# ishine/ASR-Rescoring

Hardware: AMD Instinct MI355X
Metric: masked-token BERT forwards/sec (MLM_PLL, N=50, L~32) (higher is better)
Workload: dtype fp16x3-split (fp32-accurate: hi/lo fp16 operand split on fp16 MFMA, fp32 accumulate)

## Files before the change

asr-rescoring_amd/csrc/gemm_dev.h:

```cpp
#pragma once
#include "common.h"

namespace {

typedef float f32x2 __attribute__((ext_vector_type(2)));
__device__ __forceinline__ f32x2 gelu2(f32x2 x) {
    constexpr float AMAX = 8.06101731f;
    const f32x2 a = __builtin_elementwise_min(__builtin_elementwise_abs(x), (f32x2)(AMAX));
    f32x2 q = __builtin_elementwise_fma(a, (f32x2)(3.309473686e-05f), (f32x2)(-7.692362997e-04f));
    q = __builtin_elementwise_fma(q, a, (f32x2)(8.080770262e-03f));
    q = __builtin_elementwise_fma(q, a, (f32x2)(-5.341218412e-02f));
    q = __builtin_elementwise_fma(q, a, (f32x2)(-4.587709010e-01f));
    q = __builtin_elementwise_fma(q, a, (f32x2)(-1.151201725e+00f));
    q = __builtin_elementwise_fma(q, a, (f32x2)(-9.999930859e-01f));
    const f32x2 e = {__builtin_amdgcn_exp2f(q.x), __builtin_amdgcn_exp2f(q.y)};
    const f32x2 r = x - __builtin_elementwise_min(x, (f32x2)(0.f));
    return __builtin_elementwise_fma(-a, e, r);
}

template <int E>
__device__ __forceinline__ float mix_val(unsigned hi2, unsigned lo2, float inv64) {
    float d;
    if constexpr (E == 0)
        asm("v_fma_mix_f32 %0, %1, %2, %3 op_sel_hi:[1,0,1]" : "=v"(d) : "v"(lo2), "s"(inv64), "v"(hi2));
    else
        asm("v_fma_mix_f32 %0, %1, %2, %3 op_sel:[1,0,1] op_sel_hi:[1,0,1]" : "=v"(d) : "v"(lo2), "s"(inv64), "v"(hi2));
    return d;
}
__device__ __forceinline__ unsigned mix_lo2(unsigned hi2, float x0x64, float x1x64, float neg64) {
    unsigned d;
    asm("v_fma_mixlo_f16 %0, %1, %2, %3 op_sel_hi:[1,0,0]" : "=v"(d) : "v"(hi2), "s"(neg64), "v"(x0x64));
    asm("v_fma_mixhi_f16 %0, %1, %2, %3 op_sel:[1,0,0] op_sel_hi:[1,0,0]" : "+v"(d) : "v"(hi2), "s"(neg64), "v"(x1x64));
    return d;
}

template <bool NT>
__device__ __forceinline__ void st16(uint4* p, uint4 v) {
    typedef unsigned int u32x4 __attribute__((ext_vector_type(4)));
    if constexpr (NT) __builtin_nontemporal_store((u32x4){v.x, v.y, v.z, v.w}, (u32x4*)p);
    else *p = v;
}

__device__ __forceinline__ int g16(int rb) { return (0x78 >> (2 * (rb & 3))) & 3; }

__device__ __forceinline__ void slab_read4(const char* slb, int rr0, int c16, uint4 (&v)[4]) {
    const uint32_t base = (uint32_t)(uintptr_t)(const __attribute__((address_space(3))) char*)slb;
    uint32_t a[4];
#pragma unroll
    for (int it = 0; it < 4; ++it) {
        const int rr = it * 8 + rr0;
        a[it] = base + rr * 128 + ((c16 ^ (rr & 7)) << 4);
    }
    uint4 v0, v1, v2, v3;
    asm volatile(
        "ds_read_b128 %0, %4\n\t"
        "ds_read_b128 %1, %5\n\t"
        "ds_read_b128 %2, %6\n\t"
        "ds_read_b128 %3, %7\n\t"
        "s_waitcnt lgkmcnt(0)"
        : "=&v"(v0), "=&v"(v1), "=&v"(v2), "=&v"(v3)
        : "v"(a[0]), "v"(a[1]), "v"(a[2]), "v"(a[3])
        : "memory");
    v[0] = v0; v[1] = v1; v[2] = v2; v[3] = v3;
}

}
```

asr-rescoring_amd/csrc/k_gemm.hip:

```cpp
#include <atomic>
#include "common.h"
#include "gemm_dev.h"

#ifndef RS_DIAG
#define RS_DIAG 0
#endif
#include <stdio.h>
#include <stdlib.h>
#include <string.h>
#include <type_traits>

namespace {

enum : int {
    P_SCHED = 1 << 18,
    P_SLAB = 1 << 20,
    P_X3IMG = 1 << 22,
    P_TAG_OPROJ = 1 << 16,
    P_TAG_FFN2 = 1 << 17,
    X_GANG_XCD = 1 << 27,
    X_TAG_FFN2 = 1 << 26,
    X_DIAG_NOSTAGE = 1,
    X_DIAG_NOSTORE = 2,
    X_DIAG_NOWAIT = 8,
// ... 674 lines not shown

__device__ __forceinline__ unsigned long long lnr_wait_ticks(int diag) { return (diag & 8) ? 1000ull : 100000000ull; }
__device__ __forceinline__ unsigned long long lnr_form_ticks(int diag) { return (diag & 8) ? 1000ull : 1000000000ull; }
__device__ __forceinline__ unsigned long long lnr_now() { return __builtin_amdgcn_s_memrealtime(); }

typedef __attribute__((address_space(1))) unsigned lgu32;
typedef __attribute__((address_space(1))) unsigned long long lgu64;
__device__ __forceinline__ unsigned lnr_add(unsigned* c, int w, unsigned v = 1u) {
    return __hip_atomic_fetch_add((lgu32*)(c + w), v, __ATOMIC_RELAXED, __HIP_MEMORY_SCOPE_AGENT);
}
__device__ __forceinline__ unsigned lnr_ld(const unsigned* c, int w) {
    return __hip_atomic_load((const lgu32*)(c + w), __ATOMIC_RELAXED, __HIP_MEMORY_SCOPE_AGENT);
}

constexpr unsigned LNR_PENDING = 0xfffffffeu, LNR_CANCELLED = 0xffffffffu;
constexpr unsigned long long LNR_CANCEL_TICKS = 5000ull;
template <bool XCD>
__device__ unsigned lnr_gang_ticket(const EpiArgs& ep, int ntn_, int n_panels) {
    unsigned* c = ep.lncnt;
    const unsigned ntn = (unsigned)ntn_, G = gridDim.x;
    const unsigned long long tag = (unsigned long long)ep.ln_tag << 32;
    unsigned long long* tab = (unsigned long long*)c + LNC_TAB;
    const unsigned long long t_lim = lnr_form_ticks(ep.diag), t_start = lnr_now();
    auto ld64 = [](unsigned long long* p) {
        return __hip_atomic_load((const lgu64*)p, __ATOMIC_RELAXED, __HIP_MEMORY_SCOPE_AGENT);
    };
    auto cas64 = [](unsigned long long* p, unsigned long long& expect, unsigned long long want) {
        return __hip_atomic_compare_exchange_strong((lgu64*)p, &expect, want, __ATOMIC_RELAXED, __ATOMIC_RELAXED,
                                                    __HIP_MEMORY_SCOPE_AGENT);
    };
    const unsigned NL = min(G / ntn, (unsigned)n_panels);
    auto exhausted = [&]() { return lnr_ld(c, LNC_GANGS) >= NL; };
    auto complete = [&](unsigned long long* slot, unsigned& gid) -> bool {
        unsigned long long v = ld64(slot);
        for (;;) {
            if ((v >> 32) == (tag >> 32)) return false;
            if (cas64(slot, v, tag | LNR_PENDING)) break;
        }
        gid = lnr_add(c, LNC_GANGS);
        __hip_atomic_store((lgu64*)slot, tag | gid, __ATOMIC_RELAXED, __HIP_MEMORY_SCOPE_AGENT);
        return true;
    };
    auto await_id = [&](unsigned long long* slot, bool local, unsigned& gid) -> int {
        const unsigned long long t0 = lnr_now();
        for (unsigned spins = 1;; ++spins) {
            unsigned long long v = ld64(slot);
            if ((v >> 32) == (tag >> 32)) {
                const unsigned st = (unsigned)v;
                if (st == LNR_CANCELLED) return -1;
                if (st != LNR_PENDING) {
                    gid = st;
                    return 1;
                }
            } else if ((local && lnr_now() - t0 > ((ep.diag & 8) ? 0ull : LNR_CANCEL_TICKS)) || exhausted()) {
                if (cas64(slot, v, tag | LNR_CANCELLED)) return -1;
                continue;
            }
            if ((spins & 63) == 0 && (lnr_now() - t_start > t_lim || lnr_ld(ep.lnerr, 0))) return 0;
            __builtin_amdgcn_s_sleep(1);
        }
    };
    unsigned gid = 0, mem = 0;
    bool ovf = !XCD, ok = true;
    if constexpr (XCD) {
        unsigned x;
        asm volatile("s_getreg_b32 %0, hwreg(HW_REG_XCC_ID)" : "=s"(x));
        x &= 7;
        const unsigned cap = (G / 8) / ntn * ntn;
        const unsigned lc = lnr_add(c, LNC_LOCAL + 16 * (int)x);
        ovf = lc >= cap;
        if (!ovf) {
            const unsigned k = lc / ntn;
            mem = lc - k * ntn;
            unsigned long long* slot = tab + x * 128 + k;
            if (mem + 1 == ntn) {
                ovf = !complete(slot, gid);
            } else {
                const int r = await_id(slot, true, gid);
                ok = r != 0;
                ovf = r < 0;
            }
        }
    }
    if (ovf && ok) {
        const unsigned o = lnr_add(c, LNC_OVF), k = o / ntn;
        mem = o - k * ntn;
        unsigned long long* slot = tab + 8 * 128 + k;
        if (k >= 256) {
            ok = false;
        } else if (mem + 1 == ntn) {
            if (!complete(slot, gid)) gid = NL;
        } else {
            const int r = await_id(slot, false, gid);
            ok = r != 0;
            if (r < 0) gid = NL;
        }
    }
    if (!ok) {
        __hip_atomic_store((lgu32*)ep.lnerr, 1u, __ATOMIC_RELAXED, __HIP_MEMORY_SCOPE_AGENT);
        return 0xffffffffu;
    }
    return gid >= NL ? 0xfffffffeu : gid * ntn + mem;
}

__device__ __forceinline__ bool lnr_next_list(const EpiArgs& ep, int& t, unsigned nlist, int p, int tcol, int ntn,
                                              int n_tiles, int wave, int lane) {
    const int n_panels = n_tiles / ntn;
    const unsigned NL = min((unsigned)(gridDim.x / ntn), (unsigned)n_panels);
    const unsigned long long tag = (unsigned long long)ep.ln_tag << 32;
    unsigned long long* clm = (unsigned long long*)ep.lnx + (size_t)n_panels * ntn * 512 + p;
    if (tcol == 0 && wave == 0 && lane == 0)
        __hip_atomic_store((lgu64*)clm, tag | nlist, __ATOMIC_RELAXED, __HIP_MEMORY_SCOPE_AGENT);
    const unsigned long long t_lim = lnr_wait_ticks(ep.diag), t_start = lnr_now();
    for (unsigned spins = 1;; ++spins) {
        const unsigned long long v = __hip_atomic_load((const lgu64*)clm, __ATOMIC_RELAXED, __HIP_MEMORY_SCOPE_AGENT);
        if ((v >> 32) == (tag >> 32) && !(ep.diag & 8)) {
            const unsigned l = (unsigned)v;
            t = l < NL ? (int)l * ntn + tcol : n_tiles;
            return true;
        }
        if ((spins & 63) == 0 && (lnr_now() - t_start > t_lim || lnr_ld(ep.lnerr, 0))) {
            if (lane == 0) __hip_atomic_store((lgu32*)ep.lnerr, 1u, __ATOMIC_RELAXED, __HIP_MEMORY_SCOPE_AGENT);
            return false;
        }
        __builtin_amdgcn_s_sleep(1);
    }
}

__device__ __forceinline__ void lnr_done(const EpiArgs& ep, int lane) {
    unsigned* c = ep.lncnt;
    unsigned last = 0;
    if (lane == 0) last = lnr_add(c, LNC_DONE) + 1 == gridDim.x;
    if (!__builtin_amdgcn_readfirstlane(last)) return;
    static_assert(LNC_TAB_N % 64 == 0, "gang slots per lane");
    unsigned long long* tab = (unsigned long long*)c + LNC_TAB;
#pragma unroll
    for (int i = 0; i < LNC_TAB_N / 64; ++i)
        __hip_atomic_store((lgu64*)(tab + lane + 64 * i), 0ull, __ATOMIC_RELAXED, __HIP_MEMORY_SCOPE_AGENT);
    if (lane != 0) return;
    const int w[] = {LNC_OVF, LNC_GANGS, LNC_DONE};
    for (int x = 0; x < 8; ++x) __hip_atomic_store((lgu32*)(c + LNC_LOCAL + 16 * x), 0u, __ATOMIC_RELAXED, __HIP_MEMORY_SCOPE_AGENT);
    for (int i = 0; i < 3; ++i) __hip_atomic_store((lgu32*)(c + w[i]), 0u, __ATOMIC_RELAXED, __HIP_MEMORY_SCOPE_AGENT);
}

template <int EPI, int OPT>
__global__ void __launch_bounds__(512)
gemm_x3s_kernel(const f16* __restrict__ A, const f16* __restrict__ W, int K, int ldw, int n_tiles_n, int n_tiles,
                EpiArgs ep) {
    constexpr int BM = 256, BK = 32, NW = 8, WN = 4, WTM = 128, WTN = 64;
    constexpr int RB = BK * 2;
    constexpr int REG = BM * RB;
    constexpr int STAGE = 4 * REG;
    constexpr int NSTORE = 32;
    static_assert(EPI == EPI_BIAS_F32 || EPI == EPI_GELU_F16 || EPI == EPI_LNRES_IMG, "x3s epilogues");
    constexpr bool LNR = EPI == EPI_LNRES_IMG;
    constexpr int DV = RS_DIAG ? OPT & (X_DIAG_NOSTAGE | X_DIAG_NOSTORE | X_DIAG_NOWAIT | X_DIAG_PANEL0 | X_DIAG_STAMP) : 0;
    static_assert(!LNR || (DV & X_DIAG_NOSTORE) == 0, "the LayerNorm epilogue has no no-store diagnostic");
    constexpr bool STAMP = (DV & X_DIAG_STAMP) != 0;
    unsigned long long st_sum[10] = {0, 0, 0, 0, 0, 0, 0, 0, 0, 0}, st_prev = 0;
    auto stamp = [&](int ph) __attribute__((always_inline)) {
        if constexpr (STAMP) {
            unsigned long long tt;
            __builtin_amdgcn_sched_barrier(0);
            asm volatile("s_memtime %0\n\ts_waitcnt lgkmcnt(0)" : "=s"(tt)::"memory");
            __builtin_amdgcn_sched_barrier(0);
            if (ph >= 0) st_sum[ph] += tt - st_prev;
            st_prev = tt;
        }
    };
    stamp(-1);
    extern __shared__ __attribute__((aligned(16))) char smem[];
    __shared__ __attribute__((aligned(16))) char slabs[NW * 4096];

    const int tid = threadIdx.x, lane = tid & 63;
    const int wave = __builtin_amdgcn_readfirstlane(tid >> 6);
    const int wm = wave / WN, wn = wave % WN;
    const int nk = K / BK;
    int t = blockIdx.x;
    typedef __attribute__((address_space(1))) unsigned gu32;
    typedef __attribute__((address_space(1))) unsigned long long gu64;
    if constexpr (LNR) {
        if (tid == 0) *(unsigned*)(slabs + 2048) = lnr_gang_ticket<(OPT & X_GANG_XCD) != 0>(ep, n_tiles_n, n_tiles / n_tiles_n);
        __syncthreads();
        t = (int)*(const unsigned*)(slabs + 2048);
    }
    stamp(8);
    if ((unsigned)t >= (unsigned)n_tiles) {
        if constexpr (LNR) {
            if (wave == 0) lnr_done(ep, lane);
        }
        return;
    }
    if (wave >= NW / 2) __builtin_amdgcn_s_setprio(1);
    auto tile_of = [&](int tt, int& m0, int& n0) {
        if constexpr (LNR) {
            m0 = (tt / n_tiles_n) * BM;
            n0 = (tt - (tt / n_tiles_n) * n_tiles_n) * BM;
            return;
        }
        const int xcd = tt & 7, pos = tt >> 3, q = n_tiles >> 3, r = n_tiles & 7;
        const int wgid = (xcd < r ? xcd * (q + 1) : r * (q + 1) + (xcd - r) * q) + pos;
        const int GM = ep.group_m, n_tiles_m = n_tiles / n_tiles_n, per_group = GM * n_tiles_n;
        const int g = wgid / per_group, loc = wgid - g * per_group;
        const int gm = min(GM, n_tiles_m - g * GM);
        const int tn = loc / gm;
        m0 = (g * GM + (loc - tn * gm)) * BM;
        n0 = tn * BM;
    };
    const size_t ld2 = (size_t)2 * K;
    __amdgpu_buffer_rsrc_t rsA, rsW;
    int voffA[4], voffW[4];
    auto wperm = [](int L) {
        return LNR ? (L & ~31) | (((L >> 2) & 3) << 3) | (((L >> 4) & 1) << 2) | (L & 3) : L;
    };
#pragma unroll
    for (int h = 0; h < 2; ++h)
#pragma unroll
        for (int l = 0; l < 2; ++l) {
            const int n = 128 * h + wave * 16 + 8 * l + (lane >> 3);
            const int sl = ((lane & 7) ^ ((n >> 1) & 7)) * 8;
            voffA[2 * h + l] = (n * (int)ld2 + sl) * 2;
            voffW[2 * h + l] = (wperm(n) * ldw + sl) * 2;
        }
    auto set_rsrc = [&](int m0, int n0) {
        rsA = __builtin_amdgcn_make_buffer_rsrc((void*)(A + (size_t)m0 * ld2), (short)0, (int)(256 * ld2 * 2), 0x00020000);
        rsW = __builtin_amdgcn_make_buffer_rsrc((void*)(W + (size_t)n0 * ldw), (short)0, 256 * ldw * 2, 0x00020000);
    };
    auto piece = [&](int buf, int k0, int p) {
        if constexpr ((DV & X_DIAG_NOSTAGE) != 0) return;
        const int r = p >> 1;
        const int dofs = (r >> 1) * 2 * REG + ((p & 1) * 128 + wave * 16 + 8 * (r & 1)) * 128;
        auto* dst = (__attribute__((address_space(3))) void*)(smem + buf * STAGE + dofs);
        const int vo = (r < 2 ? voffA : voffW)[2 * (p & 1) + (r & 1)];
        __builtin_amdgcn_raw_ptr_buffer_load_lds(r < 2 ? rsA : rsW, dst, 16, vo, k0 * 4, 0, 0);
    };
    auto stage = [&](int buf, int k0) {
#pragma unroll
        for (int p = 0; p < 8; ++p) piece(buf, k0, p);
    };
    const half8 up = (half8)(f16)X3_UP;

    const int r16 = lane & 15, q4 = lane >> 4;
    const int offA16 = (wm * WTM + r16) * 128 + ((q4 ^ ((r16 >> 1) & 7)) << 4);
    const int offW16 = 2 * REG + (wn * WTN + r16) * 128 + ((q4 ^ ((r16 >> 1) & 7)) << 4);
    f32x4 acc16[8][4];
    auto kstep16 = [&](int buf, int k0n) {
        const char* sb = smem + buf * STAGE;
        half8 wh[4], wl[4], wu[4];
#pragma unroll
        for (int j = 0; j < 4; ++j) {
            wh[j] = *(const half8*)(sb + offW16 + j * 2048);
            wl[j] = *(const half8*)(sb + (offW16 ^ 64) + j * 2048);
        }
#pragma unroll
        for (int j = 0; j < 4; ++j) wu[j] = wh[j] * up;
#pragma unroll
        for (int h = 0; h < 2; ++h) {
            half8 ah[4], al[4];
#pragma unroll
            for (int ii = 0; ii < 4; ++ii) {
                ah[ii] = *(const half8*)(sb + offA16 + (4 * h + ii) * 2048);
                al[ii] = *(const half8*)(sb + (offA16 ^ 64) + (4 * h + ii) * 2048);
            }
#pragma unroll
            for (int pr = 0; pr < 3; ++pr) {
#pragma unroll
                for (int ii = 0; ii < 4; ++ii) {
#pragma unroll
                    for (int j = 0; j < 4; ++j) {
                        const half8 b = pr == 0 ? wu[j] : pr == 1 ? wh[j] : wl[j];
                        const half8 a = pr == 1 ? al[ii] : ah[ii];
                        acc16[4 * h + ii][j] = __builtin_amdgcn_mfma_f32_16x16x32_f16(b, a, acc16[4 * h + ii][j], 0, 0, 0);
                    }
                    const int grp = 12 * h + 4 * pr + ii;
                    if (grp < 8 && k0n < (1 << 29)) {
                        __builtin_amdgcn_sched_barrier(0);
                        piece(buf ^ 1, k0n, grp);
                        __builtin_amdgcn_sched_barrier(0);
                    }
                }
            }
        }
    };

    int m0, n0;
    tile_of(t, m0, n0);
    set_rsrc(m0, n0);
    stage(0, 0);
    int par = 0;
    bool first = true;
    for (;;) {
        unsigned nlist = 0;
        if constexpr (LNR) {
            if (m0 / BM + (int)gridDim.x / n_tiles_n >= n_tiles / n_tiles_n && n0 == 0 && wave == 0 && lane == 0)
                nlist = lnr_add(ep.lncnt, LNC_GANGS);
        }
#pragma unroll
        for (int i = 0; i < 8; ++i)
#pragma unroll
            for (int j = 0; j < 4; ++j) acc16[i][j] = (f32x4)(0.f);
        int kt0 = 0;
        if constexpr (LNR) {
            if constexpr ((DV & X_DIAG_NOWAIT) == 0) {
                if (!first) asm volatile("s_waitcnt vmcnt(%0)" ::"n"(NSTORE) : "memory");
                else asm volatile("s_waitcnt vmcnt(0)" ::: "memory");
            }
            asm volatile("s_barrier" ::: "memory");
            __builtin_amdgcn_sched_barrier(0);
            kstep16(par, BK);
            __builtin_amdgcn_sched_barrier(0);
            stamp(9);
            kt0 = 1;
        }
        for (int kt = kt0; kt < nk; ++kt) {
            const int cur = (par + kt) & 1;
            if constexpr ((DV & X_DIAG_NOWAIT) != 0) {
            } else if (kt == 0 && !first) asm volatile("s_waitcnt vmcnt(%0)" ::"n"(NSTORE) : "memory");
            else asm volatile("s_waitcnt vmcnt(0)" ::: "memory");
            asm volatile("s_barrier" ::: "memory");
            __builtin_amdgcn_sched_barrier(0);
            kstep16(cur, kt + 1 < nk ? (kt + 1) * BK : (1 << 29));
            __builtin_amdgcn_sched_barrier(0);
            if constexpr (STAMP && !LNR) {
                if (kt == 0) stamp(9);
            }
        }
        stamp(0);
        const int last = (par + nk - 1) & 1;
        const int cm0 = m0, cn0 = n0;
        const int rbo = (last ^ 1) * STAGE + wave * 8192;
        const __amdgpu_buffer_rsrc_t rsR = __builtin_amdgcn_make_buffer_rsrc(
            (void*)((const f16*)ep.out + (size_t)cm0 * ep.ldc), (short)0, 256 * ep.ldc * 2, 0x00020000);
        int voR[4];
#pragma unroll
        for (int q = 0; q < 4; ++q) {
            const int jr = 8 * (q & 1) + (lane >> 3);
            const int cc = (lane & 7) ^ ((jr >> 1) & 7);
            voR[q] = ((wm * WTM + jr) * ep.ldc + 2 * (cn0 + wn * WTN) + 64 * (q >> 1) + 8 * cc) * 2;
        }
        auto issue = [&](int rb) __attribute__((always_inline)) {
#pragma unroll
            for (int q = 0; q < 4; ++q) {
                auto* dst = (__attribute__((address_space(3))) void*)(smem + rbo + (rb & 1) * 4096 + q * 1024);
                __builtin_amdgcn_raw_ptr_buffer_load_lds(rsR, dst, 16, voR[q], rb * 16 * ep.ldc * 2, 0, 0);
            }
        };
        if constexpr (LNR) {
            issue(0);
            issue(1);
        }
        f32x4 bq[4];
#pragma unroll
        for (int j = 0; j < 4; ++j) {
            const float* bp = ep.bias + cn0 + wn * WTN + (LNR ? 32 * (j >> 1) + 8 * q4 + 4 * (j & 1) : 16 * j + 4 * q4);
            asm volatile("global_load_dwordx4 %0, %1, off" : "=v"(bq[j]) : "v"(bp) : "memory");
        }
        asm volatile("s_waitcnt vmcnt(0)" : "+v"(bq[0]), "+v"(bq[1]), "+v"(bq[2]), "+v"(bq[3]) : : "memory");
        bool more = false;
        t += gridDim.x;
        if constexpr (LNR) {
            if (t >= n_tiles && !lnr_next_list(ep, t, nlist, cm0 / BM, cn0 / BM, n_tiles_n, n_tiles, wave, lane)) break;
        }
        more = t < n_tiles;
        if (more) {
            tile_of(t, m0, n0);
            set_rsrc(m0, n0);
            if constexpr (!LNR) stage(last ^ 1, 0);
        }
        stamp(1);
        auto finish = [&](int i0, int i1) {
#pragma unroll
            for (int i = i0; i < i1; ++i)
#pragma unroll
                for (int j = 0; j < 4; ++j)
#pragma unroll
                    for (int e = 0; e < 4; e += 2) {
                        f32x2 v = __builtin_elementwise_fma((f32x2){acc16[i][j][e], acc16[i][j][e + 1]}, (f32x2)(X3_DOWN),
                                                            (f32x2){bq[j][e], bq[j][e + 1]});
                        if constexpr (EPI == EPI_GELU_F16) v = gelu2(v);
                        acc16[i][j][e] = v.x;
                        acc16[i][j][e + 1] = v.y;
                    }
        };
            auto lnres_epilogue = [&]() {
                const int H = ep.nlog, ntn = n_tiles_n;
                const int panel = cm0 / BM, tcol = cn0 / BM;
                const unsigned long long tag = (unsigned long long)ep.ln_tag << 32;
                auto add_res = [&](int rb, const half4 (&rh)[4], const half4 (&rl)[4]) __attribute__((always_inline)) {
#pragma unroll
                    for (int j = 0; j < 4; ++j) {
                        const uint2 hv = __builtin_bit_cast(uint2, rh[j]), lv = __builtin_bit_cast(uint2, rl[j]);
                        const float hres[4] = {mix_val<0>(hv.x, lv.x, X3_DOWN), mix_val<1>(hv.x, lv.x, X3_DOWN),
                                               mix_val<0>(hv.y, lv.y, X3_DOWN), mix_val<1>(hv.y, lv.y, X3_DOWN)};
#pragma unroll
                        for (int e = 0; e < 4; ++e)
                            acc16[rb][j][e] = __builtin_fmaf(acc16[rb][j][e], X3_DOWN, bq[j][e]) + hres[e];
                    }
                };
                {
                    const uint32_t lrow = (uint32_t)(uintptr_t)(const __attribute__((address_space(3))) char*)smem + rbo +
                                          r16 * 128;
                    const uint32_t lh = lrow + ((q4 ^ ((r16 >> 1) & 7)) << 4), ll = lrow + (((q4 + 4) ^ ((r16 >> 1) & 7)) << 4);
#pragma unroll
                    for (int rb = 0; rb < 8; ++rb) {
                        if (rb < 7) asm volatile("s_waitcnt vmcnt(4)" ::: "memory");
                        else asm volatile("s_waitcnt vmcnt(0)" ::: "memory");
                        uint4 h0, h1, l0, l1;
                        const int so = (rb & 1) * 4096;
                        asm volatile(
                            "ds_read_b128 %0, %4 offset:%6\n\t"
                            "ds_read_b128 %1, %4 offset:%7\n\t"
                            "ds_read_b128 %2, %5 offset:%6\n\t"
                            "ds_read_b128 %3, %5 offset:%7\n\t"
                            "s_waitcnt lgkmcnt(0)"
                            : "=&v"(h0), "=&v"(h1), "=&v"(l0), "=&v"(l1)
                            : "v"(lh), "v"(ll), "i"(so), "i"(so + 2048)
                            : "memory");
                        if (rb + 2 < 8) issue(rb + 2);
                        const half8 vh0 = __builtin_bit_cast(half8, h0), vh1 = __builtin_bit_cast(half8, h1);
                        const half8 vl0 = __builtin_bit_cast(half8, l0), vl1 = __builtin_bit_cast(half8, l1);
                        const half4 rh[4] = {(half4){vh0[0], vh0[1], vh0[2], vh0[3]}, (half4){vh0[4], vh0[5], vh0[6], vh0[7]},
                                             (half4){vh1[0], vh1[1], vh1[2], vh1[3]}, (half4){vh1[4], vh1[5], vh1[6], vh1[7]}};
                        const half4 rl[4] = {(half4){vl0[0], vl0[1], vl0[2], vl0[3]}, (half4){vl0[4], vl0[5], vl0[6], vl0[7]},
                                             (half4){vl1[0], vl1[1], vl1[2], vl1[3]}, (half4){vl1[4], vl1[5], vl1[6], vl1[7]}};
                        add_res(rb, rh, rl);
                    }
                }
                stamp(2);
                float* red = (float*)(slabs + wave * 4096);
                auto slab_of = [&](int w2) { return (const float*)(slabs + (wm * WN + w2) * 4096); };
                float tmean[8];
#pragma unroll
                for (int i = 0; i < 8; ++i) {
                    float a = 0.f;
#pragma unroll
                    for (int j = 0; j < 4; ++j) a += (acc16[i][j][0] + acc16[i][j][1]) + (acc16[i][j][2] + acc16[i][j][3]);
                    a += __shfl_xor(a, 16);
                    a += __shfl_xor(a, 32);
                    tmean[i] = a;
                }
                if (q4 == 0) {
#pragma unroll
                    for (int i = 0; i < 8; ++i) red[16 * i + r16] = tmean[i];
                }
                asm volatile("s_waitcnt lgkmcnt(0)\n\ts_barrier" ::: "memory");
#pragma unroll
                for (int i = 0; i < 8; ++i) {
                    float a = 0.f;
#pragma unroll
                    for (int w2 = 0; w2 < WN; ++w2) a += slab_of(w2)[16 * i + r16];
                    tmean[i] = a * (1.f / BM);
                }
#pragma unroll
                for (int i = 0; i < 8; ++i) {
                    float q = 0.f;
#pragma unroll
                    for (int j = 0; j < 4; ++j)
#pragma unroll
                        for (int e = 0; e < 4; ++e) {
                            const float d = acc16[i][j][e] - tmean[i];
                            q = __builtin_fmaf(d, d, q);
                        }
                    q += __shfl_xor(q, 16);
                    q += __shfl_xor(q, 32);
                    if (q4 == 0) red[128 + 16 * i + r16] = q;
                }
                asm volatile("s_waitcnt lgkmcnt(0)\n\ts_barrier" ::: "memory");
                float2* st2 = (float2*)(smem + last * STAGE) + wm * WTM;
                volatile unsigned* bailw = (volatile unsigned*)(smem + last * STAGE + 4096);
                if (wn == 0) {
                    typedef unsigned long long u64;
                    u64* gx = (u64*)ep.lnx + (size_t)panel * ntn * BM * 2 + wm * WTM * 2;
                    int ln = lane;
                    asm volatile("" : "+v"(ln));
                    float os[2], oq[2];
#pragma unroll
                    for (int k = 0; k < 2; ++k) {
                        const int rr = ln + 64 * k;
                        float a = 0.f, b = 0.f;
#pragma unroll
                        for (int w2 = 0; w2 < WN; ++w2) {
                            a += slab_of(w2)[rr];
                            b += slab_of(w2)[128 + rr];
                        }
                        os[k] = a;
                        oq[k] = b;
                        u64* g = gx + ((size_t)tcol * BM + rr) * 2;
                        __hip_atomic_store((gu64*)g, tag | __float_as_uint(a), __ATOMIC_RELAXED, __HIP_MEMORY_SCOPE_AGENT);
                        __hip_atomic_store((gu64*)(g + 1), tag | __float_as_uint(b), __ATOMIC_RELAXED, __HIP_MEMORY_SCOPE_AGENT);
                    }
                    float ps[2][4], pq[2][4];
                    bool failed = false;
                    stamp(3);
                    const unsigned long long t_lim = lnr_wait_ticks(ep.diag), t_start = lnr_now();
                    for (unsigned spins = 0;;) {
                        bool ok = true;
#pragma unroll
                        for (int k = 0; k < 2; ++k)
#pragma unroll
                            for (int c = 0; c < 4; ++c) {
                                ps[k][c] = os[k];
                                pq[k][c] = oq[k];
                                if (c < ntn && c != tcol) {
                                    const u64* g = gx + ((size_t)c * BM + ln + 64 * k) * 2;
                                    const u64 va = __hip_atomic_load((const gu64*)g, __ATOMIC_RELAXED, __HIP_MEMORY_SCOPE_AGENT);
                                    const u64 vb = __hip_atomic_load((const gu64*)(g + 1), __ATOMIC_RELAXED, __HIP_MEMORY_SCOPE_AGENT);
                                    ok &= (va >> 32) == (tag >> 32) && (vb >> 32) == (tag >> 32);
                                    ps[k][c] = __uint_as_float((unsigned)va);
                                    pq[k][c] = __uint_as_float((unsigned)vb);
                                }
                            }
                        if (ep.diag & 8) ok = false;
                        if (__all(ok)) break;
                        __builtin_amdgcn_s_sleep(1);
                        if ((++spins & 63) == 0 &&
                            (lnr_now() - t_start > t_lim ||
                             __hip_atomic_load((const gu32*)ep.lnerr, __ATOMIC_RELAXED, __HIP_MEMORY_SCOPE_AGENT))) {
                            if (lane == 0) __hip_atomic_store((gu32*)ep.lnerr, 1u, __ATOMIC_RELAXED, __HIP_MEMORY_SCOPE_AGENT);
                            failed = true;
                            break;
                        }
                    }
#pragma unroll
                    for (int k = 0; k < 2; ++k) {
                        const float inv_n = 1.f / H;
                        float tot = 0.f;
#pragma unroll
                        for (int c = 0; c < 4; ++c)
                            if (c < ntn) tot += ps[k][c];
                        const float mean = tot * inv_n;
                        float m2 = 0.f;
#pragma unroll
                        for (int c = 0; c < 4; ++c) {
                            if (c < ntn) {
                                const float d = ps[k][c] * (1.f / BM) - mean;
                                m2 += __builtin_fmaf((float)BM * d, d, pq[k][c]);
                            }
                        }
                        st2[lane + 64 * k] = make_float2(mean, 1.0f / sqrtf(__builtin_fmaf(m2, inv_n, ep.ln_eps)));
                    }
                    if (lane == 0) bailw[wm] = failed ? 1u : 0u;
                    stamp(4);
                }
                asm volatile("s_waitcnt lgkmcnt(0)\n\ts_barrier" ::: "memory");
                if (bailw[0] | bailw[1]) return true;
                f32x4 gq[4], bb[4];
#pragma unroll
                for (int j = 0; j < 4; ++j) {
                    const int cj = cn0 + wn * WTN + 32 * (j >> 1) + 8 * q4 + 4 * (j & 1);
                    gq[j] = *(const f32x4*)(ep.res_g + cj);
                    bb[j] = *(const f32x4*)(ep.res_b + cj);
                }
#pragma unroll
                for (int i = 0; i < 8; ++i) {
                    const float2 st = st2[16 * i + r16];
#pragma unroll
                    for (int j = 0; j < 4; ++j)
#pragma unroll
                        for (int e = 0; e < 4; ++e) acc16[i][j][e] = ln_apply(acc16[i][j][e], st, gq[j][e], bb[j][e]);
                }
                stamp(5);
                return false;
            };
            constexpr bool LATE = EPI == EPI_GELU_F16 && (DV & X_DIAG_NOSTORE) == 0;
            if constexpr (LNR) {
                if (lnres_epilogue()) {
                    asm volatile("s_waitcnt vmcnt(0)" ::: "memory");
                    break;
                }
                if (more) stage(last ^ 1, 0);
            } else if constexpr (!LATE) finish(0, 8);
            if constexpr ((DV & X_DIAG_NOSTORE) != 0) {
#pragma unroll
                for (int i = 0; i < 8; ++i)
#pragma unroll
                    for (int j = 0; j < 4; ++j) asm volatile("" ::"v"(acc16[i][j]));
                if (!more) break;
                par = last ^ 1;
                first = false;
                continue;
            }
            char* slb = slabs + wave * 4096;
            int lns = lane;
            if constexpr (LNR) asm volatile("" : "+v"(lns));
            const int rr0 = lns >> 3, c16 = lns & 7;
            const int sm0 = (DV & X_DIAG_PANEL0) ? 0 : cm0;
            if constexpr (EPI == EPI_BIAS_F32) {
#pragma unroll
                for (int i2 = 0; i2 < 4; ++i2)
#pragma unroll
                    for (int j2 = 0; j2 < 2; ++j2) {
#pragma unroll
                        for (int a = 0; a < 2; ++a)
#pragma unroll
                            for (int b = 0; b < 2; ++b) {
                                const int row = 16 * a + r16, ch = 4 * b + q4;
                                *(f32x4*)(slb + row * 128 + ((ch ^ (row & 7)) << 4)) = acc16[2 * i2 + a][2 * j2 + b];
                            }
                        float* ob = (float*)ep.out + (size_t)(sm0 + wm * WTM + 32 * i2) * ep.ldc + cn0 + wn * WTN + 32 * j2 + 4 * c16;
                        uint4 v[4];
                        slab_read4(slb, rr0, c16, v);
#pragma unroll
                        for (int it = 0; it < 4; ++it) st16<true>((uint4*)(ob + (size_t)(it * 8 + rr0) * ep.ldc), v[it]);
                    }
            } else {
#pragma unroll
                for (int i2 = 0; i2 < 4; ++i2) {
                    if constexpr (LATE) finish(2 * i2, 2 * i2 + 2);
#pragma unroll
                    for (int g = 0; g < 2; ++g) {
#pragma unroll
                        for (int a = 0; a < 2; ++a)
#pragma unroll
                            for (int jj = 0; jj < 2; ++jj) {
                                half4 hh, hl;
                                const f32x4 xv = acc16[2 * i2 + a][2 * g + jj];
#pragma unroll
                                for (int e = 0; e < 4; ++e) hh[e] = (f16)xv[e];
                                const uint2 hv = __builtin_bit_cast(uint2, hh);
                                const f32x2 s01 = (f32x2){xv[0], xv[1]} * X3_UP, s23 = (f32x2){xv[2], xv[3]} * X3_UP;
                                hl = __builtin_bit_cast(half4, (uint2){mix_lo2(hv.x, s01.x, s01.y, -X3_UP),
                                                                       mix_lo2(hv.y, s23.x, s23.y, -X3_UP)});
                                const int row = 16 * a + r16, byte = LNR ? 16 * q4 + 8 * jj : 32 * jj + 8 * q4;
                                *(half4*)(slb + row * 128 + (((byte >> 4) ^ (row & 7)) << 4) + (byte & 8)) = hh;
                                *(half4*)(slb + row * 128 + ((((byte >> 4) + 4) ^ (row & 7)) << 4) + (byte & 8)) = hl;
                            }
                        f16* ob = (f16*)ep.out + (size_t)(sm0 + wm * WTM + 32 * i2) * ep.ldc + 2 * (cn0 + wn * WTN) + 64 * g + 8 * c16;
                        uint4 v[4];
                        slab_read4(slb, rr0, c16, v);
#pragma unroll
                        for (int it = 0; it < 4; ++it) st16<true>((uint4*)(ob + (size_t)(it * 8 + rr0) * ep.ldc), v[it]);
                    }
                }
            }
            stamp(6);
            if constexpr (STAMP) st_sum[7] += 1;
            if (!more) break;
            par = last ^ 1;
            first = false;
    }
    if constexpr (STAMP) {
        if (tid == 0) {
#pragma unroll
            for (int ph = 0; ph < 10; ++ph) ep.dbg[blockIdx.x * 16 + ph] += st_sum[ph];
        }
    }
    if constexpr (LNR) {
        if (wave == 0) lnr_done(ep, lane);
    }
}

unsigned ln_tag_next() {
    static std::atomic<unsigned> seq{0};
    unsigned v = seq.fetch_add(1, std::memory_order_relaxed) + 1;
    while (v == 0) v = seq.fetch_add(1, std::memory_order_relaxed) + 1;
    return v;
}

int n_cus() {
    static int n = [] {
        int dev = 0, v = 0;
        (void)hipGetDevice(&dev);
        (void)hipDeviceGetAttribute(&v, hipDeviceAttributeMultiprocessorCount, dev);
        return v > 0 ? v : 256;
    }();
    return n;
}

hipError_t smem_attr_once(const void* fn, int smem, std::atomic<unsigned>& devs) {
    int dev = 0;
    if (hipError_t e = hipGetDevice(&dev)) return e;
    const unsigned bit = 1u << (dev & 31);
    if (devs.load(std::memory_order_acquire) & bit) return hipSuccess;
    if (hipError_t e = hipFuncSetAttribute(fn, hipFuncAttributeMaxDynamicSharedMemorySize, smem)) return e;
    devs.fetch_or(bit, std::memory_order_release);
    return hipSuccess;
}

template <int EPI, int OPT = 0>
hipError_t launch_x3s(const f16* A, const f16* W, int M_pad, int N_pad, int K, const EpiArgs& ep, hipStream_t st,
                      int ldw = 0) {
    constexpr int smem = 2 * 65536;
    if (K % 32 || K < 64 || M_pad % 256 || N_pad % 256) return hipErrorInvalidValue;
    static std::atomic<unsigned> attr_devs{0};
    if (hipError_t e = smem_attr_once((const void*)gemm_x3s_kernel<EPI, OPT>, smem, attr_devs)) return e;
    const int ntn = N_pad / 256, n_tiles = (M_pad / 256) * ntn;
    const int cus = n_cus() / 8 * 8;
    int grid = n_tiles <= cus ? n_tiles : cus;
    if constexpr (EPI == EPI_LNRES_IMG) {
        if (!ep.lnx || !ep.lncnt || !ep.lnerr || N_pad > 1024 || ep.nlog != N_pad || ep.ldc != 2 * N_pad)
            return hipErrorInvalidValue;
        grid = std::min(n_tiles, cus / ntn * ntn);
    }
    static const int gm_env = getenv("RS_GEMM_GROUP_M_X3S") ? atoi(getenv("RS_GEMM_GROUP_M_X3S")) : 0;
    EpiArgs e2 = ep;
    e2.group_m = gm_env > 0 ? gm_env : 8;
    if constexpr (EPI == EPI_LNRES_IMG) {
        e2.ln_tag = ln_tag_next();
    }
    const int ldw2 = ldw > 0 ? ldw : 2 * K;
    hipLaunchKernelGGL((gemm_x3s_kernel<EPI, OPT>), dim3(grid), dim3(512), smem, st, A, W, K, ldw2, ntn, n_tiles, e2);
    return hipGetLastError();
}

template <int EPI, int OPT = 0>
hipError_t launch_persist(const f16* A, const f16* W, int M_pad, int N_pad, int K, const EpiArgs& ep,
                          hipStream_t st) {
    constexpr int smem = 2 * 512 * 64 * 2 + ((OPT & P_SLAB) ? 8 * 32 * 128 : 0);
    if (K % 64 || M_pad % 256 || N_pad % 256) return hipErrorInvalidValue;
    static std::atomic<unsigned> attr_devs{0};
    if (hipError_t e = smem_attr_once((const void*)gemm_persist_kernel<EPI, OPT>, smem, attr_devs)) return e;
    const int ntn = N_pad / 256, n_tiles = (M_pad / 256) * ntn;
    const int cus = n_cus() / 8 * 8;
    const int grid = n_tiles <= cus ? n_tiles : cus;
    static const int gm_env = getenv("RS_GEMM_GROUP_M_P") ? atoi(getenv("RS_GEMM_GROUP_M_P")) : 0;
    static const int gm_ffn2 = getenv("RS_GEMM_GROUP_M_FFN2") ? atoi(getenv("RS_GEMM_GROUP_M_FFN2")) : 0;
    EpiArgs e2 = ep;
    e2.group_m = (OPT & P_TAG_FFN2) && gm_ffn2 > 0 ? gm_ffn2 : gm_env > 0 ? gm_env : 8;
    hipLaunchKernelGGL((gemm_persist_kernel<EPI, OPT>), dim3(grid), dim3(512), smem, st, A, W, K, ntn, n_tiles, e2);
    return hipGetLastError();
}

template <int EPI, int V>
hipError_t persist_tagged(int tag, const f16* A, const f16* W, int M_pad, int N_pad, int K, const EpiArgs& ep,
                          hipStream_t st) {
    return tag == 1 ? launch_persist<EPI, V | P_TAG_OPROJ>(A, W, M_pad, N_pad, K, ep, st)
         : tag == 2 ? launch_persist<EPI, V | P_TAG_FFN2>(A, W, M_pad, N_pad, K, ep, st)
                    : launch_persist<EPI, V>(A, W, M_pad, N_pad, K, ep, st);
}

template <int BM, int BN, int WM, int WN, int NSTAGE, int BK, int EPI>
hipError_t launch_t(const f16* A, const f16* W, int M_pad, int N_pad, int K, const EpiArgs& ep,
                    hipStream_t st) {
    constexpr int smem = NSTAGE * (BM + BN) * BK * 2;
    if (K % BK) return hipErrorInvalidValue;
    static std::atomic<unsigned> attr_devs{0};
    if (hipError_t e = smem_attr_once((const void*)gemm_f16_kernel<BM, BN, WM, WN, NSTAGE, BK, EPI>, smem, attr_devs)) return e;
    const int ntn = N_pad / BN;
    const int grid = (M_pad / BM) * ntn;
    static const int gm_env = getenv("RS_GEMM_GROUP_M") ? atoi(getenv("RS_GEMM_GROUP_M")) : 0;
    EpiArgs e2 = ep;
    e2.group_m = gm_env > 0 ? gm_env : 4;
    hipLaunchKernelGGL((gemm_f16_kernel<BM, BN, WM, WN, NSTAGE, BK, EPI>), dim3(grid), dim3(WM * WN * 64),
                       smem, st, A, W, K, ntn, e2);
    return hipGetLastError();
}

template <int EPI>
hipError_t launch_epi(const f16* A, const f16* W, int M_pad, int N_pad, int K, const EpiArgs& ep,
                      hipStream_t st, int tag) {
    const bool n256 = N_pad % 256 == 0;
    if constexpr (EPI == EPI_GELU_F16) {
        if (n256 && ep.kx == 3) return launch_persist<EPI, P_SCHED | P_X3IMG>(A, W, M_pad, N_pad, K, ep, st);
    }
    if constexpr (EPI == EPI_BIAS_F16 || EPI == EPI_GELU_F16) {
        if (n256 && (EPI == EPI_BIAS_F16 || ep.kx == 1)) {
            constexpr int SLAB = EPI == EPI_BIAS_F16 ? P_SLAB : 0;
            return persist_tagged<EPI, P_SCHED | SLAB>(tag, A, W, M_pad, N_pad, K, ep, st);
        }
    }
    if (n256) return launch_t<256, 256, 2, 4, 2, 64, EPI>(A, W, M_pad, N_pad, K, ep, st);
    return launch_t<256, 128, 4, 2, 3, 64, EPI>(A, W, M_pad, N_pad, K, ep, st);
}

}

int gemm_row_align() { return 256; }

size_t lnres_counter_bytes() { return lnr_counter_bytes(); }

int gemm_lnres_workgroups(int N_pad) {
    const int ntn = N_pad / 256, cus = n_cus() / 8 * 8;
    return ntn > 0 ? cus / ntn * ntn : 0;
}

#if RS_DIAG
static unsigned long long* g_stamps = nullptr;
constexpr int STAMP_WORDS = 4 * 256 * 16;
#endif

template <int STV>
hipError_t launch_gemm_x3s_v(int epi, const f16* A, const f16* W, int ldw, int M_pad, int N_pad, int K,
                             const EpiArgs& ep_in, hipStream_t st) {
    EpiArgs ep = ep_in;
#if RS_DIAG
    if (STV) ep.dbg = g_stamps + (epi == EPI_BIAS_F32 ? 0 : epi == EPI_GELU_F16 ? 1 : K > 1024 ? 3 : 2) * 256 * 16;
#endif
    switch (epi) {
        case EPI_BIAS_F32: return launch_x3s<EPI_BIAS_F32, STV>(A, W, M_pad, N_pad, K, ep, st, ldw);
        case EPI_GELU_F16: return launch_x3s<EPI_GELU_F16, STV>(A, W, M_pad, N_pad, K, ep, st, ldw);
        case EPI_LNRES_IMG: {
            const char* g = getenv("RS_LNGANG");
            const bool xcd = !(g && !strcmp(g, "ticket"));
            if (xcd) {
                if (K > 1024) return launch_x3s<EPI_LNRES_IMG, STV | X_TAG_FFN2 | X_GANG_XCD>(A, W, M_pad, N_pad, K, ep, st, ldw);
                return launch_x3s<EPI_LNRES_IMG, STV | X_GANG_XCD>(A, W, M_pad, N_pad, K, ep, st, ldw);
            }
// ... 215 lines not shown
```

Baseline: 68870.

## Prefetch epilogue vectors into LDS and pipeline slab writes with reads and stores

The per-tile bias, LayerNorm gamma and beta vectors are now loaded asynchronously into per-wave LDS with buffer_load_lds at tile start, and the epilogue reads them from LDS. Before, it issued global loads and waited on vmcnt(0) in the middle of the epilogue. The epilogue store loop is restructured into a 16-block software pipeline across two slab halves: the next block's writes overlap the outstanding ds_read of the current block, using partial lgkmcnt waits. The aim is to hide global-load latency for the vectors and LDS round-trip latency in the epilogue. The cost is more intricate waitcnt accounting, with the NSTORE+NVEC counts, which is fragile.

```diff
diff --git a/asr-rescoring_amd/csrc/gemm_dev.h b/asr-rescoring_amd/csrc/gemm_dev.h
--- a/asr-rescoring_amd/csrc/gemm_dev.h
+++ b/asr-rescoring_amd/csrc/gemm_dev.h
@@ -43,25 +43,28 @@
 
 __device__ __forceinline__ int g16(int rb) { return (0x78 >> (2 * (rb & 3))) & 3; }
 
-__device__ __forceinline__ void slab_read4(const char* slb, int rr0, int c16, uint4 (&v)[4]) {
-    const uint32_t base = (uint32_t)(uintptr_t)(const __attribute__((address_space(3))) char*)slb;
-    uint32_t a[4];
-#pragma unroll
-    for (int it = 0; it < 4; ++it) {
-        const int rr = it * 8 + rr0;
-        a[it] = base + rr * 128 + ((c16 ^ (rr & 7)) << 4);
-    }
-    uint4 v0, v1, v2, v3;
+typedef unsigned int u32x2 __attribute__((ext_vector_type(2)));
+typedef unsigned int u32x4 __attribute__((ext_vector_type(4)));
+__device__ __forceinline__ uint32_t lds_addr(const char* p) {
+    return (uint32_t)(uintptr_t)(const __attribute__((address_space(3))) char*)p;
+}
+__device__ __forceinline__ void slab_write8(uint32_t a, u32x2 v, int half) {
+    asm volatile("ds_write_b64 %0, %1 offset:%2" : : "v"(a), "v"(v), "i"(half) : "memory");
+}
+__device__ __forceinline__ void slab_write16(uint32_t a, u32x4 v, int half) {
+    asm volatile("ds_write_b128 %0, %1 offset:%2" : : "v"(a), "v"(v), "i"(half) : "memory");
+}
+__device__ __forceinline__ void slab_read2_issue(uint32_t a, int half, u32x4& v0, u32x4& v1) {
     asm volatile(
-        "ds_read_b128 %0, %4\n\t"
-        "ds_read_b128 %1, %5\n\t"
-        "ds_read_b128 %2, %6\n\t"
-        "ds_read_b128 %3, %7\n\t"
-        "s_waitcnt lgkmcnt(0)"
-        : "=&v"(v0), "=&v"(v1), "=&v"(v2), "=&v"(v3)
-        : "v"(a[0]), "v"(a[1]), "v"(a[2]), "v"(a[3])
+        "ds_read_b128 %0, %2 offset:%3\n\t"
+        "ds_read_b128 %1, %2 offset:%4"
+        : "=&v"(v0), "=&v"(v1)
+        : "v"(a), "i"(half), "i"(half + 1024)
         : "memory");
-    v[0] = v0; v[1] = v1; v[2] = v2; v[3] = v3;
+}
+template <int N>
+__device__ __forceinline__ void slab_read2_wait(u32x4& v0, u32x4& v1) {
+    asm volatile("s_waitcnt lgkmcnt(%2)" : "+v"(v0), "+v"(v1) : "n"(N) : "memory");
 }
 
 }
diff --git a/asr-rescoring_amd/csrc/k_gemm.hip b/asr-rescoring_amd/csrc/k_gemm.hip
--- a/asr-rescoring_amd/csrc/k_gemm.hip
+++ b/asr-rescoring_amd/csrc/k_gemm.hip
@@ -850,12 +850,13 @@
     constexpr int REG = BM * RB;
     constexpr int STAGE = 4 * REG;
     constexpr int NSTORE = 32;
+    constexpr int NVEC = EPI == EPI_LNRES_IMG ? 3 : 1;
     static_assert(EPI == EPI_BIAS_F32 || EPI == EPI_GELU_F16 || EPI == EPI_LNRES_IMG, "x3s epilogues");
     constexpr bool LNR = EPI == EPI_LNRES_IMG;
     constexpr int DV = RS_DIAG ? OPT & (X_DIAG_NOSTAGE | X_DIAG_NOSTORE | X_DIAG_NOWAIT | X_DIAG_PANEL0 | X_DIAG_STAMP) : 0;
     static_assert(!LNR || (DV & X_DIAG_NOSTORE) == 0, "the LayerNorm epilogue has no no-store diagnostic");
     constexpr bool STAMP = (DV & X_DIAG_STAMP) != 0;
-    unsigned long long st_sum[10] = {0, 0, 0, 0, 0, 0, 0, 0, 0, 0}, st_prev = 0;
+    unsigned long long st_sum[15] = {0, 0, 0, 0, 0, 0, 0, 0, 0, 0, 0, 0, 0, 0, 0}, st_prev = 0;
     auto stamp = [&](int ph) __attribute__((always_inline)) {
         if constexpr (STAMP) {
             unsigned long long tt;
@@ -878,9 +879,9 @@
     typedef __attribute__((address_space(1))) unsigned gu32;
     typedef __attribute__((address_space(1))) unsigned long long gu64;
     if constexpr (LNR) {
-        if (tid == 0) *(unsigned*)(slabs + 2048) = lnr_gang_ticket<(OPT & X_GANG_XCD) != 0>(ep, n_tiles_n, n_tiles / n_tiles_n);
+        if (tid == 0) *(unsigned*)slabs = lnr_gang_ticket<(OPT & X_GANG_XCD) != 0>(ep, n_tiles_n, n_tiles / n_tiles_n);
         __syncthreads();
-        t = (int)*(const unsigned*)(slabs + 2048);
+        t = (int)*(const unsigned*)slabs;
     }
     stamp(8);
     if ((unsigned)t >= (unsigned)n_tiles) {
@@ -994,13 +995,20 @@
                 nlist = lnr_add(ep.lncnt, LNC_GANGS);
         }
 #pragma unroll
+        for (int v = 0; v < NVEC; ++v) {
+            const float* vec = (v == 0 ? ep.bias : v == 1 ? ep.res_g : ep.res_b) + n0 + wn * WTN;
+            const __amdgpu_buffer_rsrc_t rsV = __builtin_amdgcn_make_buffer_rsrc((void*)vec, (short)0, 256, 0x00020000);
+            __builtin_amdgcn_raw_ptr_buffer_load_lds(rsV, (__attribute__((address_space(3))) void*)(slabs + wave * 4096 + 1024 * (v + 1)),
+                                                     16, (lane & 15) * 16, 0, 0, 0);
+        }
+#pragma unroll
         for (int i = 0; i < 8; ++i)
 #pragma unroll
             for (int j = 0; j < 4; ++j) acc16[i][j] = (f32x4)(0.f);
         int kt0 = 0;
         if constexpr (LNR) {
             if constexpr ((DV & X_DIAG_NOWAIT) == 0) {
-                if (!first) asm volatile("s_waitcnt vmcnt(%0)" ::"n"(NSTORE) : "memory");
+                if (!first) asm volatile("s_waitcnt vmcnt(%0)" ::"n"(NSTORE + NVEC) : "memory");
                 else asm volatile("s_waitcnt vmcnt(0)" ::: "memory");
             }
             asm volatile("s_barrier" ::: "memory");
@@ -1013,7 +1021,7 @@
         for (int kt = kt0; kt < nk; ++kt) {
             const int cur = (par + kt) & 1;
             if constexpr ((DV & X_DIAG_NOWAIT) != 0) {
-            } else if (kt == 0 && !first) asm volatile("s_waitcnt vmcnt(%0)" ::"n"(NSTORE) : "memory");
+            } else if (kt == 0 && !first) asm volatile("s_waitcnt vmcnt(%0)" ::"n"(NSTORE + NVEC) : "memory");
             else asm volatile("s_waitcnt vmcnt(0)" ::: "memory");
             asm volatile("s_barrier" ::: "memory");
             __builtin_amdgcn_sched_barrier(0);
@@ -1047,13 +1055,22 @@
             issue(0);
             issue(1);
         }
+        const uint32_t bqa = lds_addr(slabs + wave * 4096 + 1024) + (LNR ? 32 : 16) * q4;
+        auto slab_vec = [&](int vec, f32x4 (&q)[4]) __attribute__((always_inline)) {
+            asm volatile(
+                "ds_read_b128 %0, %4 offset:%5\n\t"
+                "ds_read_b128 %1, %4 offset:%6\n\t"
+                "ds_read_b128 %2, %4 offset:%7\n\t"
+                "ds_read_b128 %3, %4 offset:%8\n\t"
+                "s_waitcnt lgkmcnt(0)"
+                : "=&v"(q[0]), "=&v"(q[1]), "=&v"(q[2]), "=&v"(q[3])
+                : "v"(bqa), "i"(1024 * vec), "i"(1024 * vec + (LNR ? 16 : 64)), "i"(1024 * vec + 128),
+                  "i"(1024 * vec + (LNR ? 144 : 192))
+                : "memory");
+        };
         f32x4 bq[4];
-#pragma unroll
-        for (int j = 0; j < 4; ++j) {
-            const float* bp = ep.bias + cn0 + wn * WTN + (LNR ? 32 * (j >> 1) + 8 * q4 + 4 * (j & 1) : 16 * j + 4 * q4);
-            asm volatile("global_load_dwordx4 %0, %1, off" : "=v"(bq[j]) : "v"(bp) : "memory");
-        }
-        asm volatile("s_waitcnt vmcnt(0)" : "+v"(bq[0]), "+v"(bq[1]), "+v"(bq[2]), "+v"(bq[3]) : : "memory");
+        slab_vec(0, bq);
+        stamp(14);
         bool more = false;
         t += gridDim.x;
         if constexpr (LNR) {
@@ -1066,11 +1083,11 @@
             if constexpr (!LNR) stage(last ^ 1, 0);
         }
         stamp(1);
-        auto finish = [&](int i0, int i1) {
+        auto finish = [&](int i0, int i1, int j0, int j1) __attribute__((always_inline)) {
 #pragma unroll
             for (int i = i0; i < i1; ++i)
 #pragma unroll
-                for (int j = 0; j < 4; ++j)
+                for (int j = j0; j < j1; ++j)
 #pragma unroll
                     for (int e = 0; e < 4; e += 2) {
                         f32x2 v = __builtin_elementwise_fma((f32x2){acc16[i][j][e], acc16[i][j][e + 1]}, (f32x2)(X3_DOWN),
@@ -1243,12 +1260,8 @@
                 asm volatile("s_waitcnt lgkmcnt(0)\n\ts_barrier" ::: "memory");
                 if (bailw[0] | bailw[1]) return true;
                 f32x4 gq[4], bb[4];
-#pragma unroll
-                for (int j = 0; j < 4; ++j) {
-                    const int cj = cn0 + wn * WTN + 32 * (j >> 1) + 8 * q4 + 4 * (j & 1);
-                    gq[j] = *(const f32x4*)(ep.res_g + cj);
-                    bb[j] = *(const f32x4*)(ep.res_b + cj);
-                }
+                slab_vec(1, gq);
+                slab_vec(2, bb);
 #pragma unroll
                 for (int i = 0; i < 8; ++i) {
                     const float2 st = st2[16 * i + r16];
@@ -1267,7 +1280,10 @@
                     break;
                 }
                 if (more) stage(last ^ 1, 0);
-            } else if constexpr (!LATE) finish(0, 8);
+            } else if constexpr (!LATE) {
+                finish(0, 8, 0, 4);
+                stamp(10);
+            }
             if constexpr ((DV & X_DIAG_NOSTORE) != 0) {
 #pragma unroll
                 for (int i = 0; i < 8; ++i)
@@ -1283,53 +1299,70 @@
             if constexpr (LNR) asm volatile("" : "+v"(lns));
             const int rr0 = lns >> 3, c16 = lns & 7;
             const int sm0 = (DV & X_DIAG_PANEL0) ? 0 : cm0;
-            if constexpr (EPI == EPI_BIAS_F32) {
-#pragma unroll
-                for (int i2 = 0; i2 < 4; ++i2)
-#pragma unroll
-                    for (int j2 = 0; j2 < 2; ++j2) {
-#pragma unroll
-                        for (int a = 0; a < 2; ++a)
-#pragma unroll
-                            for (int b = 0; b < 2; ++b) {
-                                const int row = 16 * a + r16, ch = 4 * b + q4;
-                                *(f32x4*)(slb + row * 128 + ((ch ^ (row & 7)) << 4)) = acc16[2 * i2 + a][2 * j2 + b];
-                            }
-                        float* ob = (float*)ep.out + (size_t)(sm0 + wm * WTM + 32 * i2) * ep.ldc + cn0 + wn * WTN + 32 * j2 + 4 * c16;
-                        uint4 v[4];
-                        slab_read4(slb, rr0, c16, v);
-#pragma unroll
-                        for (int it = 0; it < 4; ++it) st16<true>((uint4*)(ob + (size_t)(it * 8 + rr0) * ep.ldc), v[it]);
-                    }
-            } else {
-#pragma unroll
-                for (int i2 = 0; i2 < 4; ++i2) {
-                    if constexpr (LATE) finish(2 * i2, 2 * i2 + 2);
-#pragma unroll
-                    for (int g = 0; g < 2; ++g) {
-#pragma unroll
-                        for (int a = 0; a < 2; ++a)
-#pragma unroll
-                            for (int jj = 0; jj < 2; ++jj) {
-                                half4 hh, hl;
-                                const f32x4 xv = acc16[2 * i2 + a][2 * g + jj];
-#pragma unroll
-                                for (int e = 0; e < 4; ++e) hh[e] = (f16)xv[e];
-                                const uint2 hv = __builtin_bit_cast(uint2, hh);
-                                const f32x2 s01 = (f32x2){xv[0], xv[1]} * X3_UP, s23 = (f32x2){xv[2], xv[3]} * X3_UP;
-                                hl = __builtin_bit_cast(half4, (uint2){mix_lo2(hv.x, s01.x, s01.y, -X3_UP),
-                                                                       mix_lo2(hv.y, s23.x, s23.y, -X3_UP)});
-                                const int row = 16 * a + r16, byte = LNR ? 16 * q4 + 8 * jj : 32 * jj + 8 * q4;
-                                *(half4*)(slb + row * 128 + (((byte >> 4) ^ (row & 7)) << 4) + (byte & 8)) = hh;
-                                *(half4*)(slb + row * 128 + ((((byte >> 4) + 4) ^ (row & 7)) << 4) + (byte & 8)) = hl;
-                            }
-                        f16* ob = (f16*)ep.out + (size_t)(sm0 + wm * WTM + 32 * i2) * ep.ldc + 2 * (cn0 + wn * WTN) + 64 * g + 8 * c16;
-                        uint4 v[4];
-                        slab_read4(slb, rr0, c16, v);
-#pragma unroll
-                        for (int it = 0; it < 4; ++it) st16<true>((uint4*)(ob + (size_t)(it * 8 + rr0) * ep.ldc), v[it]);
-                    }
-                }
+            constexpr int NWR = EPI == EPI_GELU_F16 ? 4 : 2;
+            const uint32_t sb = lds_addr(slb);
+            const uint32_t rda = sb + rr0 * 128 + ((c16 ^ rr0) << 4);
+            const int wo = r16 * 128 + ((((EPI == EPI_BIAS_F32 || LNR) ? q4 : q4 >> 1) ^ (r16 & 7)) << 4) +
+                           ((EPI == EPI_BIAS_F32 || LNR) ? 0 : 8 * (q4 & 1));
+            auto put_block = [&](int b) __attribute__((always_inline)) {
+                const int i = 2 * (b >> 2) + (b & 1), c = (b >> 1) & 1, half = (b & 1) * 2048;
+                if constexpr (EPI == EPI_BIAS_F32) {
+#pragma unroll
+                    for (int bb = 0; bb < 2; ++bb)
+                        slab_write16(sb + (wo ^ (64 * bb)), __builtin_bit_cast(u32x4, acc16[i][2 * c + bb]), half);
+                } else {
+                    if constexpr (LATE) {
+                        finish(i, i + 1, 2 * c, 2 * c + 2);
+                        stamp(10);
+                    }
+                    u32x2 hv[2], lv[2];
+#pragma unroll
+                    for (int jj = 0; jj < 2; ++jj) {
+                        half4 hh;
+                        const f32x4 xv = acc16[i][2 * c + jj];
+#pragma unroll
+                        for (int e = 0; e < 4; ++e) hh[e] = (f16)xv[e];
+                        hv[jj] = __builtin_bit_cast(u32x2, hh);
+                        const f32x2 s01 = (f32x2){xv[0], xv[1]} * X3_UP, s23 = (f32x2){xv[2], xv[3]} * X3_UP;
+                        lv[jj] = (u32x2){mix_lo2(hv[jj].x, s01.x, s01.y, -X3_UP), mix_lo2(hv[jj].y, s23.x, s23.y, -X3_UP)};
+                    }
+                    if constexpr (LNR) {
+                        slab_write16(sb + wo, (u32x4){hv[0].x, hv[0].y, hv[1].x, hv[1].y}, half);
+                        slab_write16(sb + (wo ^ 64), (u32x4){lv[0].x, lv[0].y, lv[1].x, lv[1].y}, half);
+                    } else {
+#pragma unroll
+                        for (int jj = 0; jj < 2; ++jj) {
+                            slab_write8(sb + (wo ^ (32 * jj)), hv[jj], half);
+                            slab_write8(sb + (wo ^ (32 * jj) ^ 64), lv[jj], half);
+                        }
+                    }
+                }
+                stamp(11);
+            };
+            put_block(0);
+#pragma unroll
+            for (int b = 0; b < 16; ++b) {
+                const int i2 = b >> 2, c = (b >> 1) & 1, a = b & 1;
+                u32x4 v0, v1;
+                slab_read2_issue(rda, a * 2048, v0, v1);
+                if (b + 1 < 16) {
+                    put_block(b + 1);
+                    slab_read2_wait<NWR>(v0, v1);
+                } else {
+                    slab_read2_wait<0>(v0, v1);
+                }
+                stamp(12);
+                const size_t orow = (size_t)(sm0 + wm * WTM + 32 * i2 + 16 * a + rr0) * ep.ldc;
+                if constexpr (EPI == EPI_BIAS_F32) {
+                    float* ob = (float*)ep.out + orow + cn0 + wn * WTN + 32 * c + 4 * c16;
+                    st16<true>((uint4*)ob, __builtin_bit_cast(uint4, v0));
+                    st16<true>((uint4*)(ob + (size_t)8 * ep.ldc), __builtin_bit_cast(uint4, v1));
+                } else {
+                    f16* ob = (f16*)ep.out + orow + 2 * (cn0 + wn * WTN) + 64 * c + 8 * c16;
+                    st16<true>((uint4*)ob, __builtin_bit_cast(uint4, v0));
+                    st16<true>((uint4*)(ob + (size_t)8 * ep.ldc), __builtin_bit_cast(uint4, v1));
+                }
+                stamp(13);
             }
             stamp(6);
             if constexpr (STAMP) st_sum[7] += 1;
@@ -1340,7 +1373,7 @@
     if constexpr (STAMP) {
         if (tid == 0) {
 #pragma unroll
-            for (int ph = 0; ph < 10; ++ph) ep.dbg[blockIdx.x * 16 + ph] += st_sum[ph];
+            for (int ph = 0; ph < 15; ++ph) ep.dbg[blockIdx.x * 16 + ph] += st_sum[ph];
         }
     }
     if constexpr (LNR) {
```

After: 69100, median of 6. About the same (+0.3%).
